# JingruiYu/FishBirdEyeVisualSLAM

Measured on AMD Instinct MI355X. Metric: frames/s (extract+match+pose-opt), 1280x720+512x512 pair, higher is better.
Workload: dtype u8 (extract, Hamming) + f64 (pose optimisation); 1 GPU; configs[2]: 1280x720 front + 512x512 bird pair, HIP ORB extract + M3/M9 Hamming match + PoseOptimizationWithBird (~2k front + ~1k bird edges); nfeatures=2000, parallelism=replicas x1

## Files before the change

### fishbirdeyevisualslam_amd/csrc/orb.hip

```cpp
#include <climits>

#include "fb_common.h"
#include "fb_fast_score.h"
#include "fb_primitives.h"

#include "orb_plan.h"

namespace {

constexpr int PATTERN_XY[1024] = {
#include "orb_pattern.inc"
};
constexpr int pattern_extreme(bool wantMax) {
  int m = PATTERN_XY[0];
  for (int i = 1; i < 1024; i++) m = wantMax ? (PATTERN_XY[i] > m ? PATTERN_XY[i] : m) : (PATTERN_XY[i] < m ? PATTERN_XY[i] : m);
  return m;
}
constexpr int PAT_BIAS = -pattern_extreme(false);
static_assert(PAT_BIAS >= 0 && pattern_extreme(true) + PAT_BIAS <= 255, "a pattern coordinate does not fit a biased byte");
struct PackedPattern { uint32_t test[256]; };
constexpr PackedPattern pack_pattern() {
  PackedPattern p{};
  for (int t = 0; t < 256; t++)
    for (int k = 0; k < 4; k++) p.test[t] |= (uint32_t)(PATTERN_XY[t * 4 + k] + PAT_BIAS) << (8 * k);
  return p;
}
__constant__ PackedPattern c_pattern = pack_pattern();

}

#include "orb_pyramid.inc"
#include "orb_fast.inc"
#include "orb_octree.inc"
#include "orb_describe.inc"

namespace {

struct Workspace {
  int w = 0, h = 0, batchCap = 0;
  OrbK K = {};
  int maxNodes = 0;
  size_t octreeLds = 0;
  bool rowsOK[FB_MAX_LEVELS] = {}, mergeOK[FB_MAX_LEVELS] = {};
  ResizeTabs rt[FB_MAX_LEVELS] = {};
  fb::DevBuf pyr, blur, cand, cellCand, cellCount, nodeOf, counts, lvlOut, tabs, angTab, timers;
};

}

struct fb_orb {
  fb_orb_params p;
  fb_orb_tables t;
  hipStream_t sideStream = nullptr;
  hipEvent_t evFork = nullptr, evJoin = nullptr;
  hipEvent_t evLevel[FB_MAX_LEVELS] = {};
  ~fb_orb() {
    if (evFork) (void)hipEventDestroy(evFork);
    if (evJoin) (void)hipEventDestroy(evJoin);
    for (hipEvent_t e : evLevel)
      if (e) (void)hipEventDestroy(e);
    if (sideStream) (void)hipStreamDestroy(sideStream);
  }
  int kpStride = 0;
  Workspace ws;
  const uint8_t *lastImg = nullptr;
  long long lastImgStride = 0;
  int lastPitch0 = 0;
  fb::DevBuf ownedImg;
};

namespace {

struct OrbCall {
  const uint8_t *img;
  long long imgStride;
  int pitch0, batch;
  hipStream_t s;
};

void launch_resize(fb_orb *o, int l, const OrbCall &c) {
  const Workspace &ws = o->ws;
  const OrbK &K = ws.K;
  const LevelInfo &D = K.L[l], &S = K.L[l - 1];
  const uint8_t *src = (l == 1) ? c.img : ws.pyr.as<uint8_t>() + S.off;
  const long long sstr = (l == 1) ? c.imgStride : K.pyrStride;
  const int spitch = (l == 1) ? c.pitch0 : S.pitch;
  uint8_t *dst = ws.pyr.as<uint8_t>() + D.off;
  const dim3 blk(64, 4);
  auto grid = [&](int rowsPerThread) { return dim3((D.pitch / 4 + 63) / 64, (D.h + 4 * rowsPerThread - 1) / (4 * rowsPerThread), c.batch); };
  fb::ProfScope prof_(fb::P_RESIZE, c.s);
  const bool rows = ws.rowsOK[l] && spitch >= 12 && ((reinterpret_cast<uintptr_t>(src) | (uintptr_t)spitch | (uintptr_t)sstr) & 3) == 0;
  if (rows && ws.mergeOK[l])
    k_resize_merge<<<grid(RM_ROWS), blk, 0, c.s>>>(src, sstr, S.w, S.h, spitch, dst, K.pyrStride, D.w, D.h, D.pitch, ws.rt[l]);
  else if (rows)
    k_resize_rows<<<grid(RESIZE_ROWS), blk, 0, c.s>>>(src, sstr, S.w, S.h, spitch, dst, K.pyrStride, D.w, D.h, D.pitch, ws.rt[l]);
// ... 40 lines not shown
      if (!o->evJoin) FB_HIP(hipEventCreateWithFlags(&o->evJoin, hipEventDisableTiming));
      for (int l = 1; l < FB_MAX_LEVELS; l++)
        if (!o->evLevel[l]) FB_HIP(hipEventCreateWithFlags(&o->evLevel[l], hipEventDisableTiming));
      FB_HIP(hipStreamCreateWithFlags(&o->sideStream, hipStreamNonBlocking));
    }
    sBlur = o->sideStream;
    FB_HIP(hipEventRecord(o->evFork, s));
    FB_HIP(hipStreamWaitEvent(sBlur, o->evFork, 0));
    return FB_OK;
  }

  int behind_level(int l) {
    const int nl = o->ws.K.nlevels;
    if (l + 1 < nl && !((cuts >> (l + 1)) & 1u)) return FB_OK;
    if (fork && l > 0) {
      FB_HIP(hipEventRecord(o->evLevel[l], c.s));
      FB_HIP(hipStreamWaitEvent(sBlur, o->evLevel[l], 0));
    }
    launch_blur(o, c, blurFrom, l + 1, sBlur);
    blurFrom = l + 1;
    if (fork && l + 1 == nl) FB_HIP(hipEventRecord(o->evJoin, sBlur));
    return FB_OK;
  }

  int join_before_describe(hipStream_t s) {
    if (fork) FB_HIP(hipStreamWaitEvent(s, o->evJoin, 0));
    return FB_OK;
  }
};

template <int TP>
void launch_fast(fb_orb *o, const OrbCall &c) {
  const Workspace &ws = o->ws;
  const OrbK &K = ws.K;
  fb::ProfScope prof_(TP == 44 ? fb::P_FAST : TP == 56 ? fb::P_FAST56 : fb::P_FAST72, c.s);
  const dim3 grd((K.totalGroups + 7) / 8 * 8, c.batch);
  const size_t lds = (size_t)2 * K.fastTileBytes + 2 * K.fastMaxPix;
  const auto kern = K.dbg == 20 ? k_fast<TP, true> : k_fast<TP, false>;
  kern<<<grd, 64, lds, c.s>>>(K, c.img, c.imgStride, c.pitch0, ws.pyr.as<uint8_t>(), ws.cellCand.as<uint32_t>(), ws.cellCount.as<int>());
}
void launch_fast(fb_orb *o, const OrbCall &c) {
  const OrbK &K = o->ws.K;
  if (K.totalCells == 0) return;
  if (K.fastTP == 44) launch_fast<44>(o, c);
  else if (K.fastTP == 56) launch_fast<56>(o, c);
  else launch_fast<FAST_MAX_TILE>(o, c);
}

template <int NT>
void launch_octree(fb_orb *o, const OrbCall &c) {
  const Workspace &ws = o->ws;
  int *candCount = ws.counts.as<int>(), *lvlCount = candCount + (size_t)ws.batchCap * ws.K.nlevels;
  fb::ProfScope prof_(fb::P_OCTREE, c.s);
  k_octree<NT><<<dim3(c.batch, ws.K.nlevels), NT, ws.octreeLds, c.s>>>(ws.K, ws.cellCand.as<uint32_t>(), ws.cellCount.as<int>(), ws.cand.as<uint32_t>(), candCount,
                                                                       ws.nodeOf.as<uint16_t>(), ws.lvlOut.as<uint32_t>(), lvlCount, ws.maxNodes);
}
void launch_octree(fb_orb *o, const OrbCall &c) {
  static const int octWideMax = getenv("FB_OCT_WIDE_MAX") ? atoi(getenv("FB_OCT_WIDE_MAX")) : 512;
  if (o->ws.K.nlevels * c.batch <= octWideMax) launch_octree<1024>(o, c);
  else launch_octree<256>(o, c);
}
template <int NT>
int allow_octree_lds() {
  FB_HIP(hipFuncSetAttribute(reinterpret_cast<const void *>(k_octree<NT>), hipFuncAttributeMaxDynamicSharedMemorySize, (int)OCTREE_LDS_MAX));
  return FB_OK;
}

void launch_describe(fb_orb *o, const OrbCall &c, fb_keypoint *d_keypoints, uint8_t *d_descriptors, int32_t *d_n) {
  const Workspace &ws = o->ws;
  const OrbK &K = ws.K;
  const int *lvlCount = ws.counts.as<int>() + (size_t)ws.batchCap * K.nlevels;
  fb::ProfScope prof_(fb::P_DESCRIBE, c.s);
  k_describe<<<dim3((K.descBase[K.nlevels] + 7) / 8 * 8, c.batch), 64 * DESC_WPB, 0, c.s>>>(K, c.img, c.imgStride, c.pitch0, ws.pyr.as<uint8_t>(), ws.blur.as<uint8_t>(),
                                                                                          ws.angTab.as<uint4>(), ws.lvlOut.as<uint32_t>(), lvlCount, d_keypoints,
                                                                                          d_descriptors, d_n);
}

int build_workspace(const OrbPlan &P, int batch, Workspace &ws) {
  ws.K = P.K;
  ws.K.dbg = getenv("FB_FAST_DBG") ? atoi(getenv("FB_FAST_DBG")) : 0;
  ws.maxNodes = P.maxNodes;
  ws.octreeLds = P.octreeLds;
  memcpy(ws.rowsOK, P.rowsOK, sizeof(ws.rowsOK));
  memcpy(ws.mergeOK, P.mergeOK, sizeof(ws.mergeOK));
  FB_TRY(ws.tabs.upload(P.tabBytes.data(), P.tabBytes.size()));
  for (int l = 1; l < P.K.nlevels; l++) {
    const uint8_t *base = ws.tabs.as<uint8_t>();
    ws.rt[l].xofs = reinterpret_cast<const int *>(base + P.tabOff[l][0]);
    ws.rt[l].ialpha = reinterpret_cast<const short *>(base + P.tabOff[l][1]);
    ws.rt[l].yofs = reinterpret_cast<const int *>(base + P.tabOff[l][2]);
    ws.rt[l].ibeta = reinterpret_cast<const short *>(base + P.tabOff[l][3]);
  }
  FB_TRY(ws.angTab.upload(P.angTab, sizeof(P.angTab)));
  const OrbSizes z = P.sizes(batch);
  FB_TRY(ws.pyr.alloc(z.pyr));
  FB_TRY(ws.blur.alloc(z.blur));
  FB_TRY(ws.cand.alloc(z.cand));
  FB_TRY(ws.cellCand.alloc(z.cellCand));
  FB_TRY(ws.cellCount.alloc(z.cellCount));
  FB_TRY(ws.nodeOf.alloc(z.nodeOf));
  FB_TRY(ws.counts.alloc(z.counts));
  FB_TRY(ws.timers.alloc(z.timers));
  FB_HIP(hipMemset(ws.timers.p, 0, z.timers));
  ws.K.timers = ws.timers.as<unsigned long long>();
  FB_TRY(ws.lvlOut.alloc(z.lvlOut));
  return FB_OK;
}

int prepare(fb_orb *o, int w, int h, int batch) {
  if (o->ws.w == w && o->ws.h == h && batch <= o->ws.batchCap) return FB_OK;
  OrbPlan P;
  FB_TRY(plan_orb(o->p, o->t, w, h, o->kpStride, P));
  Workspace ws;
  FB_TRY(build_workspace(P, batch, ws));
  FB_TRY(allow_octree_lds<1024>());
  FB_TRY(allow_octree_lds<256>());
  ws.w = w; ws.h = h; ws.batchCap = batch;
  o->ws = std::move(ws);
  return FB_OK;
}

}

extern "C" {

int fb_orb_capacity(const fb_orb_params *params) {
  if (!params) return FB_ERR_ARG;
  return capacity_of(*params);
}

int fb_orb_set_output_stride(fb_orb *h, int kp_stride) {
  FB_ARG(h && (kp_stride == 0 || kp_stride >= capacity_of(h->p)));
  h->kpStride = kp_stride;
  h->ws.K.kpStride = kp_stride > 0 ? kp_stride : capacity_of(h->p);
  return FB_OK;
// ... 158 lines not shown
```

### fishbirdeyevisualslam_amd/csrc/orb_octree.inc

```

namespace {

__device__ __forceinline__ int quadrant(const ONode &n, int rx, int ry) {
  const int halfX = (int)ceilf((float)(n.x1 - n.x0) / 2), halfY = (int)ceilf((float)(n.y1 - n.y0) / 2);
  const int mx = n.x0 + halfX, my = n.y0 + halfY;
  return (rx < mx ? 0 : 1) + (ry < my ? 0 : 2);
}

__device__ __forceinline__ ONode child_of(const ONode &n, int q, int cnt) {
  const int halfX = (int)ceilf((float)(n.x1 - n.x0) / 2), halfY = (int)ceilf((float)(n.y1 - n.y0) / 2);
  const int mx = n.x0 + halfX, my = n.y0 + halfY;
  ONode c;
  c.x0 = (q & 1) ? mx : n.x0;
  c.x1 = (q & 1) ? n.x1 : mx;
  c.y0 = (q & 2) ? my : n.y0;
  c.y1 = (q & 2) ? n.y1 : my;
  c.cnt = cnt;
  return c;
}

template <int NT>
__global__ __launch_bounds__(NT) void k_octree(OrbK K, const uint32_t *__restrict__ cellCand, const int *__restrict__ cellCount,
                                                uint32_t *__restrict__ cand, int *__restrict__ candCount, uint16_t *__restrict__ nodeOf,
                                                uint32_t *__restrict__ lvlOut, int *__restrict__ lvlCount, int maxNodes) {
  extern __shared__ __attribute__((aligned(16))) uint8_t smem[];
  const int l = blockIdx.y, b = blockIdx.x, tid = threadIdx.x;
  const LevelInfo &Lv = K.L[l];
  const int M = maxNodes;
  ONode *listA = reinterpret_cast<ONode *>(smem);
  ONode *listB = listA + M;
  int *ccnt = reinterpret_cast<int *>(listB + M);
  unsigned short *cpos = reinterpret_cast<unsigned short *>(ccnt + 4 * M);
  unsigned short *npos = cpos + 4 * M;
  unsigned short *order = npos + M;
  unsigned char *split = reinterpret_cast<unsigned char *>(order + M);
  unsigned long long *best = reinterpret_cast<unsigned long long *>(smem + (((size_t)(split + M - smem)) + 7 & ~(size_t)7));
  __shared__ int s_w[NT / 64], s_S, s_nexp, s_jstar;
  uint32_t *cdw = cand + (long long)b * K.candStride + Lv.candBase;
  int n;
  {
    int *offs = reinterpret_cast<int *>(smem);
    const int ncell = Lv.nCols * Lv.nRows;
    const int *cc = cellCount + (long long)b * K.totalCells + Lv.cellBase;
    const uint32_t *sp = cellCand + (long long)b * K.candStride + Lv.candBase;
    int run = 0;
    for (int c0 = 0; c0 < ncell; c0 += NT) {
      const int c = c0 + tid;
      const int v = c < ncell ? cc[c] : 0;
      int tot;
      const int ex = fb::block_excl_scan<NT>(v, s_w, &tot);
      if (c < ncell) offs[c] = run + ex;
      run += tot;
      __syncthreads();
    }
    n = run;
    if (tid == 0) { offs[ncell] = n; candCount[b * K.nlevels + l] = n; }
    __syncthreads();
    for (int k0 = tid; k0 < n; k0 += NT * 4) {
      uint32_t val[4];
#pragma unroll
      for (int u = 0; u < 4; u++) {
        const int k = min(k0 + u * NT, n - 1);
        int lo = 0, hi = ncell;
        while (hi - lo > 1) {
          const int mid = (lo + hi) >> 1;
          if (offs[mid] <= k) lo = mid; else hi = mid;
        }
        val[u] = sp[(long long)lo * Lv.slotCap + (k - offs[lo])];
      }
#pragma unroll
      for (int u = 0; u < 4; u++)
        if (k0 + u * NT < n) cdw[k0 + u * NT] = val[u];
    }
    __threadfence_block();
    __syncthreads();
  }
  const uint32_t *cd = cdw;
  uint16_t *nof = nodeOf + (long long)b * K.candStride + Lv.candBase;
  int *outCount = lvlCount + b * K.nlevels + l;
  uint32_t *out = lvlOut + (long long)b * K.outStride + Lv.outBase;
  if (n == 0 || Lv.nIni < 1) { if (tid == 0) *outCount = 0; return; }
  const int N = Lv.N;
  const int Hh = Lv.h - 2 * BORDER;
  for (int i = tid; i < Lv.nIni; i += NT) {
    ONode nd;
    nd.x0 = (short)(int)(Lv.hX * (float)i);
    nd.x1 = (short)(int)(Lv.hX * (float)(i + 1));
    nd.y0 = 0; nd.y1 = (short)Hh; nd.cnt = 0;
    listB[i] = nd;
  }
  __syncthreads();
  for (int k = tid; k < n; k += NT) {
    const int rx = (int)(cd[k] & 0xFFF) - BORDER;
    int idx = (int)((float)rx / Lv.hX);
    idx = min(idx, Lv.nIni - 1);
    nof[k] = (uint16_t)idx;
    atomicAdd(&listB[idx].cnt, 1);
  }
  __syncthreads();
  if (tid == 0) {
    int S = 0;
    for (int i = 0; i < Lv.nIni; i++) {
      npos[i] = (unsigned short)S;
      if (listB[i].cnt > 0) listA[S++] = listB[i];
    }
    s_S = S;
  }
  __syncthreads();
  for (int k = tid; k < n; k += NT) nof[k] = npos[nof[k]];
  __syncthreads();
  ONode *cur = listA, *nxt = listB;
  int S = s_S;
  bool finalPhase = false;
  for (int guard = 0; guard < 64; guard++) {
    const int prevSize = S;
    for (int i = tid; i < 4 * S; i += NT) ccnt[i] = 0;
    __syncthreads();
    for (int k0 = tid; k0 < n; k0 += NT * 4) {
      int pk[4];
      uint32_t ck[4];
#pragma unroll
      for (int u = 0; u < 4; u++) { const int kk = min(k0 + u * NT, n - 1); pk[u] = nof[kk]; ck[u] = cd[kk]; }
#pragma unroll
      for (int u = 0; u < 4; u++) {
        if (k0 + u * NT >= n) break;
        const int p = pk[u];
        const ONode nd = cur[p];
        if (nd.cnt > 1) {
          const uint32_t c = ck[u];
          atomicAdd(&ccnt[4 * p + quadrant(nd, (int)(c & 0xFFF) - BORDER, (int)((c >> 12) & 0xFFF) - BORDER)], 1);
        }
      }
    }
    __syncthreads();
    if (!finalPhase) {
      for (int p = tid; p < S; p += NT) split[p] = cur[p].cnt > 1;
    } else {
      for (int p = tid; p < S; p += NT) {
        split[p] = 0;
        const int c = cur[p].cnt;
        if (c > 1) {
          int rank = 0;
          for (int j = 0; j < S; j++) {
            const int cj = cur[j].cnt;
            if (cj > 1 && (cj > c || (cj == c && j < p))) rank++;
          }
          order[rank] = (unsigned short)p;
        }
      }
      __syncthreads();
      if (tid == 0) {
        int sz = S, j = 0;
        const int C = s_nexp;
        for (; j < C; j++) {
          const int p = order[j];
          const int kk = (ccnt[4 * p] > 0) + (ccnt[4 * p + 1] > 0) + (ccnt[4 * p + 2] > 0) + (ccnt[4 * p + 3] > 0);
          sz += kk - 1;
          split[p] = 1;
          if (sz >= N) { j++; break; }
        }
        s_jstar = j;
      }
    }
    __syncthreads();
    const int per = (S + NT - 1) / NT;
    const int a0 = min(tid * per, S), a1 = min(a0 + per, S);
    int myKids = 0, myKeep = 0;
    if (!finalPhase) {
      for (int p = a0; p < a1; p++) {
        if (split[p]) myKids += (ccnt[4 * p] > 0) + (ccnt[4 * p + 1] > 0) + (ccnt[4 * p + 2] > 0) + (ccnt[4 * p + 3] > 0);
        else myKeep++;
      }
    } else {
      const int J = s_jstar;
      const int perj = (J + NT - 1) / NT;
      const int r0 = min(tid * perj, J), r1 = min(r0 + perj, J);
      for (int r = r0; r < r1; r++) {
        const int p = order[r];
        myKids += (ccnt[4 * p] > 0) + (ccnt[4 * p + 1] > 0) + (ccnt[4 * p + 2] > 0) + (ccnt[4 * p + 3] > 0);
      }
      for (int p = a0; p < a1; p++) if (!split[p]) myKeep++;
    }
    int totalKids, totalKeep;
    const int kidsBefore = fb::block_excl_scan<NT>(myKids, s_w, &totalKids);
    const int keepBefore = fb::block_excl_scan<NT>(myKeep, s_w, &totalKeep);
    {
      int ci = kidsBefore, kp = totalKids + keepBefore;
      if (!finalPhase) {
        for (int p = a0; p < a1; p++) {
          if (split[p]) {
            for (int q = 0; q < 4; q++)
              if (ccnt[4 * p + q] > 0) {
                const int pos = totalKids - 1 - ci++;
                cpos[4 * p + q] = (unsigned short)pos;
                nxt[pos] = child_of(cur[p], q, ccnt[4 * p + q]);
              }
          } else {
            npos[p] = (unsigned short)kp;
            nxt[kp++] = cur[p];
          }
        }
      } else {
        const int J = s_jstar;
        const int perj = (J + NT - 1) / NT;
        const int r0 = min(tid * perj, J), r1 = min(r0 + perj, J);
        for (int r = r0; r < r1; r++) {
          const int p = order[r];
          for (int q = 0; q < 4; q++)
            if (ccnt[4 * p + q] > 0) {
              const int pos = totalKids - 1 - ci++;
              cpos[4 * p + q] = (unsigned short)pos;
              nxt[pos] = child_of(cur[p], q, ccnt[4 * p + q]);
            }
        }
        for (int p = a0; p < a1; p++)
          if (!split[p]) { npos[p] = (unsigned short)kp; nxt[kp++] = cur[p]; }
      }
    }
    const int Snew = totalKids + totalKeep;
    __syncthreads();
    for (int k0 = tid; k0 < n; k0 += NT * 4) {
      int pk[4];
      uint32_t ck[4];
#pragma unroll
      for (int u = 0; u < 4; u++) { const int kk = min(k0 + u * NT, n - 1); pk[u] = nof[kk]; ck[u] = cd[kk]; }
#pragma unroll
      for (int u = 0; u < 4; u++) {
        const int k = k0 + u * NT;
        if (k >= n) break;
        const int p = pk[u];
        if (split[p]) {
          const uint32_t c = ck[u];
          nof[k] = cpos[4 * p + quadrant(cur[p], (int)(c & 0xFFF) - BORDER, (int)((c >> 12) & 0xFFF) - BORDER)];
        } else nof[k] = npos[p];
      }
    }
    int myExp = 0;
    {
      const int pern = (Snew + NT - 1) / NT;
      const int n0 = min(tid * pern, Snew), n1 = min(n0 + pern, Snew);
      for (int p = n0; p < n1; p++) myExp += (p < totalKids && nxt[p].cnt > 1);
    }
    int nToExpand;
    fb::block_excl_scan<NT>(myExp, s_w, &nToExpand);
    if (tid == 0) s_nexp = nToExpand;
    __syncthreads();
    ONode *t = cur; cur = nxt; nxt = t;
    S = Snew;
    if (S >= N || S == prevSize) break;
    if (!finalPhase) {
      if (S + nToExpand * 3 > N) finalPhase = true;
    }
  }
  for (int p = tid; p < S; p += NT) best[p] = 0ull;
  __syncthreads();
  for (int k0 = tid; k0 < n; k0 += NT * 4) {
    int pk[4];
    uint32_t ck[4];
#pragma unroll
    for (int u = 0; u < 4; u++) { const int kk = min(k0 + u * NT, n - 1); pk[u] = nof[kk]; ck[u] = cd[kk]; }
#pragma unroll
    for (int u = 0; u < 4; u++) {
    const int k = k0 + u * NT;
    if (k >= n) break;
    const uint32_t c = ck[u];
    const int x = c & 0xFFF, y = (c >> 12) & 0xFFF, r = c >> 24;
    const int cellI = (y - EDGE_THRESHOLD) / Lv.hCell, cellJ = (x - EDGE_THRESHOLD) / Lv.wCell;
    const int dwid = min(Lv.wCell, Lv.w - 2 * EDGE_THRESHOLD - cellJ * Lv.wCell);
    const int inCell = (y - EDGE_THRESHOLD - cellI * Lv.hCell) * dwid + (x - EDGE_THRESHOLD - cellJ * Lv.wCell);
    const unsigned orderKey = (unsigned)(cellI * Lv.nCols + cellJ) * 4096u + (unsigned)inCell;
    const unsigned long long key = ((unsigned long long)r << 56) | ((unsigned long long)(0xFFFFFFFFu - orderKey) << 24) | (unsigned)k;
    atomicMax(&best[pk[u]], key);
    }
  }
  __syncthreads();
  for (int p = tid; p < S; p += NT) out[p] = cd[(unsigned)(best[p] & 0xFFFFFFull)];
  if (tid == 0) *outCount = S;
}

}
```

### fishbirdeyevisualslam_amd/csrc/orb_plan.h

```cpp
#ifndef FB_ORB_PLAN_H_
#define FB_ORB_PLAN_H_

#include <algorithm>
#include <cstdint>
#include <cstring>
#include <vector>

#include "../../include/fishbird.h"

#ifndef FB_HD
#define FB_HD
#endif
#include "fb_detmath.h"

namespace fb {
void set_error(const char *fmt, ...);
}

namespace {

constexpr int EDGE_THRESHOLD = 19;
constexpr int HALF_PATCH = 15;
constexpr int PATCH_SIZE = 31;
constexpr int BORDER = EDGE_THRESHOLD - 3;

constexpr int FAST_MAX_TILE = 72;
constexpr int FAST_CPW = 4;
constexpr int DESC_WPB = 4;
constexpr int DESC_KPW = 2;
constexpr int BLUR_ROWS = 32;
constexpr size_t OCTREE_LDS_MAX = 160 * 1024 - 512;
#ifdef FB_FAST_LISTHIST
#define FB_ORB_TIMER_WORDS (16 + 128)
#else
#define FB_ORB_TIMER_WORDS 16
#endif

struct LevelInfo {
  int w, h, pitch;
  long long off;
  int nCols, nRows, wCell, hCell, cellBase;
  int N;
  long long candBase;
  int candCap;
  int slotCap;
  int outBase, outCap;
  int nIni;
  float hX;
  float scale;
  int patchSize;
  long long boff;
};

struct OrbK {
  int nlevels, iniTh, minTh, totalCells, outStride, capOut;
  int kpStride;
  int fastTileBytes, fastMaxOut, fastMaxPix;
  int fastTP;
  int dbg;
  unsigned long long *timers;
  int cellBase[FB_MAX_LEVELS + 1];
  int grpBase[FB_MAX_LEVELS + 1];
  int totalGroups;
  int descBase[FB_MAX_LEVELS + 1];
  int runBase[FB_MAX_LEVELS];
  int runCap[FB_MAX_LEVELS];
  long long pyrStride;
  long long blurStride;
  int blurStrips[FB_MAX_LEVELS + 1];
  long long candStride;
  int umax[16];
  LevelInfo L[FB_MAX_LEVELS];
};

struct ResizeTabs {
  const int *xofs;
  const short *ialpha;
  const int *yofs;
  const short *ibeta;
};

struct ONode {
  short x0, y0, x1, y1;
  int cnt;
};

inline void make_tables(const fb_orb_params &p, fb_orb_tables &t) {
  memset(&t, 0, sizeof(t));
  const int nl = p.nlevels;
  t.scale_factor[0] = 1.0f;
  t.level_sigma2[0] = 1.0f;
  for (int i = 1; i < nl; i++) {
    t.scale_factor[i] = t.scale_factor[i - 1] * p.scale_factor;
    t.level_sigma2[i] = t.scale_factor[i] * t.scale_factor[i];
  }
  for (int i = 0; i < nl; i++) {
    t.inv_scale_factor[i] = 1.0f / t.scale_factor[i];
    t.inv_level_sigma2[i] = 1.0f / t.level_sigma2[i];
  }
  float factor = 1.0f / p.scale_factor;
  float nDesired = p.nfeatures * (1 - factor) / (1 - (float)pow((double)factor, (double)nl));
  int sum = 0;
  for (int l = 0; l < nl - 1; l++) {
    t.features_per_level[l] = fb_cvround(nDesired);
    sum += t.features_per_level[l];
    nDesired *= factor;
  }
  t.features_per_level[nl - 1] = std::max(p.nfeatures - sum, 0);
  int umax[HALF_PATCH + 2] = {0};
  int v, v0;
  const int vmax = fb_cvfloor(HALF_PATCH * sqrtf(2.f) / 2 + 1);
  const int vmin = fb_cvceil(HALF_PATCH * sqrtf(2.f) / 2);
  const double hp2 = HALF_PATCH * HALF_PATCH;
  for (v = 0; v <= vmax; ++v) umax[v] = fb_cvround_d(sqrt(hp2 - v * v));
  for (v = HALF_PATCH, v0 = 0; v >= vmin; --v) {
    while (umax[v0] == umax[v0 + 1]) ++v0;
    umax[v] = v0;
    ++v0;
  }
  for (int i = 0; i <= HALF_PATCH; i++) t.umax[i] = umax[i];
}

inline int capacity_of(const fb_orb_params &p) { return p.nfeatures + 8 * p.nlevels; }

struct OrbSizes {
  size_t pyr, blur, cand, cellCand, cellCount, nodeOf, counts, lvlOut, timers;
};

struct OrbPlan {
  OrbK K;
  bool rowsOK[FB_MAX_LEVELS];
  bool mergeOK[FB_MAX_LEVELS];
  std::vector<uint8_t> tabBytes;
  size_t tabOff[FB_MAX_LEVELS][4];
  uint32_t angTab[64 * 4];
  int maxNodes;
  size_t octreeLds;
  OrbSizes sizes(size_t B) const {
    OrbSizes z;
    z.pyr = B * K.pyrStride + 256;
    z.blur = B * K.blurStride + 256;
    z.cand = z.cellCand = B * K.candStride * 4 + 16;
    z.cellCount = B * (size_t)K.totalCells * 4 + 16;
    z.nodeOf = B * K.candStride * 2 + 16;
    z.counts = B * K.nlevels * 4 * 2 + FB_MAX_LEVELS * 4;
    z.lvlOut = B * K.outStride * 4 + 16;
    z.timers = FB_ORB_TIMER_WORDS * 8;
    return z;
  }
};

inline int plan_level(const fb_orb_params &p, const fb_orb_tables &t, int w, int h, int l, LevelInfo &L) {
  const float scale = t.inv_scale_factor[l];
  L.w = fb_cvround((float)w * scale);
  L.h = fb_cvround((float)h * scale);
  if (l == 0) { L.w = w; L.h = h; }
  if (L.w < 1 || L.h < 1) {
    fb::set_error("pyramid level %d of a %dx%d image is empty (scale factor %.3f, %d levels)", l, w, h, (double)p.scale_factor, p.nlevels);
    return FB_ERR_ARG;
  }
  if (L.w >= 4096 || L.h >= 4096) { fb::set_error("image too large (level %d is %dx%d, limit 4095)", l, L.w, L.h); return FB_ERR_ARG; }
  L.pitch = (L.w + 63) & ~63;
  const int maxBX = L.w - BORDER, maxBY = L.h - BORDER;
  const float width = (float)(maxBX - BORDER), height = (float)(maxBY - BORDER);
  L.nCols = (int)(width / 30.f);
  L.nRows = (int)(height / 30.f);
  if (L.nCols <= 0 || L.nRows <= 0) { L.nCols = L.nRows = 0; L.wCell = L.hCell = 1; }
  else { L.wCell = (int)ceilf(width / L.nCols); L.hCell = (int)ceilf(height / L.nRows); }
  if (L.wCell + 6 > FAST_MAX_TILE - 3 || L.hCell + 6 > FAST_MAX_TILE) { fb::set_error("FAST cell %dx%d exceeds the LDS tile", L.wCell, L.hCell); return FB_ERR_CAPACITY; }
  if (L.nCols * L.nRows >= (1 << 20)) { fb::set_error("level %d has more than 2^20 FAST cells", l); return FB_ERR_CAPACITY; }
  L.N = t.features_per_level[l];
  L.slotCap = ((L.wCell + 1) / 2) * ((L.hCell + 1) / 2);
  L.candCap = L.nCols * L.nRows * L.slotCap + 16;
  if (L.candCap >= (1 << 24)) { fb::set_error("level %d: more than 2^24 FAST candidates possible", l); return FB_ERR_CAPACITY; }
  const int Wr = maxBX - BORDER, Hr = maxBY - BORDER;
  L.nIni = (Hr > 0) ? (int)roundf((float)Wr / Hr) : 0;
  L.hX = L.nIni > 0 ? (float)Wr / L.nIni : 1.f;
  L.outCap = std::max(L.N + 3, 4 * L.nIni) + 4;
  L.scale = t.scale_factor[l];
  L.patchSize = (int)(PATCH_SIZE * t.scale_factor[l]);
  return FB_OK;
}

inline void plan_offsets(OrbPlan &P) {
  OrbK &K = P.K;
  long long pyrOff = 0, candOff = 0, blurOff = 0;
  int cells = 0, outOff = 0, strips = 0;
  P.maxNodes = 0;
  for (int l = 0; l < K.nlevels; l++) {
    LevelInfo &L = K.L[l];
// ... 62 lines not shown
    int sy = fb_cvfloor(fy);
    fy -= sy;
    yofs[dy] = sy;
    ibeta[dy * 2] = (short)fb_cvround((1.f - fy) * 2048.f);
    ibeta[dy * 2 + 1] = (short)fb_cvround(fy * 2048.f);
  }
  P.rowsOK[l] = resize_rows_ok(xofs);
  P.mergeOK[l] = P.rowsOK[l] && resize_merge_ok(yofs);
  auto append = [&](const void *src, size_t n) {
    const size_t off = (P.tabBytes.size() + 15) & ~(size_t)15;
    P.tabBytes.resize(off + n);
    memcpy(P.tabBytes.data() + off, src, n);
    return off;
  };
  P.tabOff[l][0] = append(xofs.data(), xofs.size() * 4);
  P.tabOff[l][1] = append(ialpha.data(), ialpha.size() * 2);
  P.tabOff[l][2] = append(yofs.data(), yofs.size() * 4);
  P.tabOff[l][3] = append(ibeta.data(), ibeta.size() * 2);
}

inline void plan_fast_tile(OrbK &K) {
  int tileB = 0, maxOut = 0, maxPix = 0, tpNeed = 0;
  for (int l = 0; l < K.nlevels; l++) {
    const LevelInfo &L = K.L[l];
    if (L.nCols * L.nRows == 0) continue;
    const int tpMax = (L.wCell + 6 + 3 + 3) & ~3, chMax = L.hCell + 6;
    tpNeed = std::max(tpNeed, tpMax);
    tileB = std::max(tileB, chMax);
    maxOut = std::max(maxOut, L.slotCap);
    maxPix = std::max(maxPix, L.wCell * L.hCell);
  }
  K.fastTP = tpNeed <= 44 ? 44 : tpNeed <= 56 ? 56 : FAST_MAX_TILE;
  K.fastTileBytes = (std::max(K.fastTP * tileB, 4 * ((maxOut + 3) & ~3)) + 15) & ~15;
  K.fastTileBytes = std::max(K.fastTileBytes, (21 * K.fastTP + 15) & ~15);
  K.fastMaxOut = (maxOut + 3) & ~3;
  K.fastMaxPix = (maxPix + 7) & ~7;
}

inline void plan_grids(OrbK &K) {
  int gsum = 0, wsum = 0;
  for (int l = 0; l <= FB_MAX_LEVELS; l++) {
    K.cellBase[l] = l < K.nlevels ? K.L[l].cellBase : K.totalCells;
    K.grpBase[l] = gsum;
    K.descBase[l] = wsum;
    if (l >= K.nlevels) continue;
    gsum += (K.L[l].nCols * K.L[l].nRows + FAST_CPW - 1) / FAST_CPW;
    K.runBase[l] = K.L[l].outBase;
    K.runCap[l] = K.L[l].outCap;
    wsum += (K.L[l].outCap + DESC_WPB * DESC_KPW - 1) / (DESC_WPB * DESC_KPW);
  }
  K.totalGroups = gsum;
}

inline int plan_octree_lds(OrbPlan &P) {
  const size_t M = P.maxNodes;
  size_t lds = 2 * M * sizeof(ONode) + 4 * M * 4 + 4 * M * 2 + M * 2 + M * 2 + M;
  lds = ((lds + 7) & ~(size_t)7) + M * 8 + 16;
  size_t maxCells = 0;
  for (int l = 0; l < P.K.nlevels; l++) maxCells = std::max(maxCells, (size_t)P.K.L[l].nCols * P.K.L[l].nRows);
  lds = std::max(lds, (maxCells + 1) * 4 + 16);
  if (lds > OCTREE_LDS_MAX) { fb::set_error("nfeatures too large for the LDS quadtree (%zu B)", lds); return FB_ERR_CAPACITY; }
  P.octreeLds = lds;
  return FB_OK;
}

inline void plan_angle_table(OrbPlan &P) {
  for (int lane = 0; lane < 62; lane++) {
    const int v = (lane >> 1) - 15, half = lane & 1, dmax = P.K.umax[v < 0 ? -v : v];
    for (int j = 0; j < 16; j++) {
      const int au = half ? j : 15 - j;
      const bool inc = au <= dmax && (half || au != 0);
      if (!inc) continue;
      P.angTab[lane * 4 + (j >> 2)] |= ((uint32_t)au | 0x10u) << (8 * (j & 3));
    }
  }
}

inline int plan_orb(const fb_orb_params &p, const fb_orb_tables &t, int w, int h, int kpStride, OrbPlan &out) {
  OrbPlan P;
  memset(&P.K, 0, sizeof(P.K));
  memset(P.rowsOK, 0, sizeof(P.rowsOK));
  memset(P.mergeOK, 0, sizeof(P.mergeOK));
  memset(P.tabOff, 0, sizeof(P.tabOff));
  memset(P.angTab, 0, sizeof(P.angTab));
  OrbK &K = P.K;
  K.nlevels = p.nlevels;
  K.iniTh = p.ini_th_fast;
  K.minTh = p.min_th_fast;
  K.capOut = capacity_of(p);
  K.kpStride = kpStride > 0 ? kpStride : K.capOut;
  for (int i = 0; i < 16; i++) K.umax[i] = t.umax[i];
  for (int l = 0; l < p.nlevels; l++) {
    const int rc = plan_level(p, t, w, h, l, K.L[l]);
    if (rc != FB_OK) return rc;
  }
  plan_offsets(P);
  for (int l = 1; l < p.nlevels; l++) plan_resize_tables(P, l);
  plan_fast_tile(K);
  plan_grids(K);
  const int rc = plan_octree_lds(P);
  if (rc != FB_OK) return rc;
  plan_angle_table(P);
  out = std::move(P);
  return FB_OK;
}

}

#endif
```

Before: 81590 frames/s.

## Keep octree candidates and node ids in LDS, fuse quadrant counting into remap

The quadtree distribution kernel now copies each level's candidates and node indices into LDS when they fit (up to 8192 candidates by default), so the per-round passes no longer read and write global memory. Quadrant counting for the next round is folded into the remap pass, removing one pass over the candidates per round. The serial choose loop run by thread 0 in the final phase is replaced by a block-wide scan with an atomicMin cutoff. Per-phase timers sit behind a template flag, and probe scripts are added. The cost is much more LDS per workgroup, which can lower occupancy, plus two code paths to maintain.

```diff
diff --git a/fishbirdeyevisualslam_amd/csrc/orb.hip b/fishbirdeyevisualslam_amd/csrc/orb.hip
--- a/fishbirdeyevisualslam_amd/csrc/orb.hip
+++ b/fishbirdeyevisualslam_amd/csrc/orb.hip
@@ -41,6 +41,7 @@
   OrbK K = {};
   int maxNodes = 0;
   size_t octreeLds = 0;
+  int octreeCand = 0, octreeCandNarrow = 0, octreeCandOff = 0;
   bool rowsOK[FB_MAX_LEVELS] = {}, mergeOK[FB_MAX_LEVELS] = {};
   ResizeTabs rt[FB_MAX_LEVELS] = {};
   fb::DevBuf pyr, blur, cand, cellCand, cellCount, nodeOf, counts, lvlOut, tabs, angTab, timers;
@@ -187,8 +188,11 @@
   const Workspace &ws = o->ws;
   int *candCount = ws.counts.as<int>(), *lvlCount = candCount + (size_t)ws.batchCap * ws.K.nlevels;
   fb::ProfScope prof_(fb::P_OCTREE, c.s);
-  k_octree<NT><<<dim3(c.batch, ws.K.nlevels), NT, ws.octreeLds, c.s>>>(ws.K, ws.cellCand.as<uint32_t>(), ws.cellCount.as<int>(), ws.cand.as<uint32_t>(), candCount,
-                                                                       ws.nodeOf.as<uint16_t>(), ws.lvlOut.as<uint32_t>(), lvlCount, ws.maxNodes);
+  const auto kern = ws.K.dbg >= 21 && ws.K.dbg < 21 + FB_MAX_LEVELS ? k_octree<NT, true> : k_octree<NT, false>;
+  const int cand = NT == 1024 ? ws.octreeCand : ws.octreeCandNarrow;
+  const size_t lds = (size_t)ws.octreeCandOff + (size_t)cand * 6;
+  kern<<<dim3(c.batch, ws.K.nlevels), NT, lds, c.s>>>(ws.K, ws.cellCand.as<uint32_t>(), ws.cellCount.as<int>(), ws.cand.as<uint32_t>(), candCount,
+                                                                       ws.nodeOf.as<uint16_t>(), ws.lvlOut.as<uint32_t>(), lvlCount, ws.maxNodes, cand, ws.octreeCandOff);
 }
 void launch_octree(fb_orb *o, const OrbCall &c) {
   static const int octWideMax = getenv("FB_OCT_WIDE_MAX") ? atoi(getenv("FB_OCT_WIDE_MAX")) : 512;
@@ -197,7 +201,8 @@
 }
 template <int NT>
 int allow_octree_lds() {
-  FB_HIP(hipFuncSetAttribute(reinterpret_cast<const void *>(k_octree<NT>), hipFuncAttributeMaxDynamicSharedMemorySize, (int)OCTREE_LDS_MAX));
+  FB_HIP(hipFuncSetAttribute(reinterpret_cast<const void *>(k_octree<NT, false>), hipFuncAttributeMaxDynamicSharedMemorySize, (int)OCTREE_LDS_MAX));
+  FB_HIP(hipFuncSetAttribute(reinterpret_cast<const void *>(k_octree<NT, true>), hipFuncAttributeMaxDynamicSharedMemorySize, (int)OCTREE_LDS_MAX));
   return FB_OK;
 }
 
@@ -215,7 +220,11 @@
   ws.K = P.K;
   ws.K.dbg = getenv("FB_FAST_DBG") ? atoi(getenv("FB_FAST_DBG")) : 0;
   ws.maxNodes = P.maxNodes;
-  ws.octreeLds = P.octreeLds;
+  const char *oc = getenv("FB_OCT_LDS_CAND");
+  ws.octreeCand = oc ? std::max(0, std::min(atoi(oc), P.octreeCandMax)) : P.octreeCand;
+  ws.octreeCandNarrow = oc ? ws.octreeCand : 0;
+  ws.octreeCandOff = (int)P.octreeNodeLds;
+  ws.octreeLds = octree_lds_bytes(P, ws.octreeCand);
   memcpy(ws.rowsOK, P.rowsOK, sizeof(ws.rowsOK));
   memcpy(ws.mergeOK, P.mergeOK, sizeof(ws.mergeOK));
   FB_TRY(ws.tabs.upload(P.tabBytes.data(), P.tabBytes.size()));
diff --git a/fishbirdeyevisualslam_amd/csrc/orb_octree.inc b/fishbirdeyevisualslam_amd/csrc/orb_octree.inc
--- a/fishbirdeyevisualslam_amd/csrc/orb_octree.inc
+++ b/fishbirdeyevisualslam_amd/csrc/orb_octree.inc
@@ -19,67 +19,34 @@
   return c;
 }
 
-template <int NT>
-__global__ __launch_bounds__(NT) void k_octree(OrbK K, const uint32_t *__restrict__ cellCand, const int *__restrict__ cellCount,
-                                                uint32_t *__restrict__ cand, int *__restrict__ candCount, uint16_t *__restrict__ nodeOf,
-                                                uint32_t *__restrict__ lvlOut, int *__restrict__ lvlCount, int maxNodes) {
-  extern __shared__ __attribute__((aligned(16))) uint8_t smem[];
-  const int l = blockIdx.y, b = blockIdx.x, tid = threadIdx.x;
-  const LevelInfo &Lv = K.L[l];
-  const int M = maxNodes;
-  ONode *listA = reinterpret_cast<ONode *>(smem);
-  ONode *listB = listA + M;
-  int *ccnt = reinterpret_cast<int *>(listB + M);
-  unsigned short *cpos = reinterpret_cast<unsigned short *>(ccnt + 4 * M);
-  unsigned short *npos = cpos + 4 * M;
-  unsigned short *order = npos + M;
-  unsigned char *split = reinterpret_cast<unsigned char *>(order + M);
-  unsigned long long *best = reinterpret_cast<unsigned long long *>(smem + (((size_t)(split + M - smem)) + 7 & ~(size_t)7));
-  __shared__ int s_w[NT / 64], s_S, s_nexp, s_jstar;
-  uint32_t *cdw = cand + (long long)b * K.candStride + Lv.candBase;
-  int n;
-  {
-    int *offs = reinterpret_cast<int *>(smem);
-    const int ncell = Lv.nCols * Lv.nRows;
-    const int *cc = cellCount + (long long)b * K.totalCells + Lv.cellBase;
-    const uint32_t *sp = cellCand + (long long)b * K.candStride + Lv.candBase;
-    int run = 0;
-    for (int c0 = 0; c0 < ncell; c0 += NT) {
-      const int c = c0 + tid;
-      const int v = c < ncell ? cc[c] : 0;
-      int tot;
-      const int ex = fb::block_excl_scan<NT>(v, s_w, &tot);
-      if (c < ncell) offs[c] = run + ex;
-      run += tot;
-      __syncthreads();
-    }
-    n = run;
-    if (tid == 0) { offs[ncell] = n; candCount[b * K.nlevels + l] = n; }
-    __syncthreads();
-    for (int k0 = tid; k0 < n; k0 += NT * 4) {
-      uint32_t val[4];
-#pragma unroll
-      for (int u = 0; u < 4; u++) {
-        const int k = min(k0 + u * NT, n - 1);
-        int lo = 0, hi = ncell;
-        while (hi - lo > 1) {
-          const int mid = (lo + hi) >> 1;
-          if (offs[mid] <= k) lo = mid; else hi = mid;
-        }
-        val[u] = sp[(long long)lo * Lv.slotCap + (k - offs[lo])];
-      }
-#pragma unroll
-      for (int u = 0; u < 4; u++)
-        if (k0 + u * NT < n) cdw[k0 + u * NT] = val[u];
-    }
-    __threadfence_block();
-    __syncthreads();
-  }
-  const uint32_t *cd = cdw;
-  uint16_t *nof = nodeOf + (long long)b * K.candStride + Lv.candBase;
-  int *outCount = lvlCount + b * K.nlevels + l;
-  uint32_t *out = lvlOut + (long long)b * K.outStride + Lv.outBase;
-  if (n == 0 || Lv.nIni < 1) { if (tid == 0) *outCount = 0; return; }
+struct OctLds {
+  ONode *listA, *listB;
+  int *ccnt;
+  unsigned short *cpos;
+  unsigned short *npos;
+  unsigned short *order;
+  unsigned char *split;
+  unsigned long long *best;
+};
+
+template <bool TIMED>
+struct OctTimer {
+  uint32_t mark = 0, start = 0, acc[7] = {0, 0, 0, 0, 0, 0, 0};
+  int rounds = 0;
+};
+template <>
+struct OctTimer<false> {};
+
+template <int NT, bool TIMED, bool RES, typename CandPtr, typename NodePtr>
+__device__ __forceinline__ int octree_rounds(const LevelInfo &Lv, const OctLds D, CandPtr cd, NodePtr nof, int n, uint32_t *__restrict__ out, int *s_w, int *s_S,
+                                             int *s_nexp, int *s_jstar, bool timed, OctTimer<TIMED> &T) {
+#define OCT_TICK(slot_) if constexpr (TIMED) if (timed) { __builtin_amdgcn_sched_barrier(0); const uint32_t t_ = (uint32_t)__builtin_amdgcn_s_memtime(); __builtin_amdgcn_sched_barrier(0); T.acc[slot_] += t_ - T.mark; T.mark = t_; }
+  const int tid = threadIdx.x;
+  ONode *listA = D.listA, *listB = D.listB;
+  int *ccnt = D.ccnt;
+  unsigned short *cpos = D.cpos, *npos = D.npos, *order = D.order;
+  unsigned char *split = D.split;
+  unsigned long long *best = D.best;
   const int N = Lv.N;
   const int Hh = Lv.h - 2 * BORDER;
   for (int i = tid; i < Lv.nIni; i += NT) {
@@ -104,35 +71,53 @@
       npos[i] = (unsigned short)S;
       if (listB[i].cnt > 0) listA[S++] = listB[i];
     }
-    s_S = S;
-  }
-  __syncthreads();
-  for (int k = tid; k < n; k += NT) nof[k] = npos[nof[k]];
-  __syncthreads();
+    *s_S = S;
+  }
+  __syncthreads();
+  if constexpr (RES) {
+    for (int i = tid; i < 4 * *s_S; i += NT) ccnt[i] = 0;
+    __syncthreads();
+    for (int k = tid; k < n; k += NT) {
+      const int p = npos[nof[k]];
+      nof[k] = (uint16_t)p;
+      const ONode nd = listA[p];
+      if (nd.cnt > 1) {
+        const uint32_t c = cd[k];
+        atomicAdd(&ccnt[4 * p + quadrant(nd, (int)(c & 0xFFF) - BORDER, (int)((c >> 12) & 0xFFF) - BORDER)], 1);
+      }
+    }
+  } else {
+    for (int k = tid; k < n; k += NT) nof[k] = npos[nof[k]];
+  }
+  __syncthreads();
+  OCT_TICK(1)
   ONode *cur = listA, *nxt = listB;
-  int S = s_S;
+  int S = *s_S;
   bool finalPhase = false;
   for (int guard = 0; guard < 64; guard++) {
     const int prevSize = S;
-    for (int i = tid; i < 4 * S; i += NT) ccnt[i] = 0;
-    __syncthreads();
-    for (int k0 = tid; k0 < n; k0 += NT * 4) {
-      int pk[4];
-      uint32_t ck[4];
-#pragma unroll
-      for (int u = 0; u < 4; u++) { const int kk = min(k0 + u * NT, n - 1); pk[u] = nof[kk]; ck[u] = cd[kk]; }
-#pragma unroll
-      for (int u = 0; u < 4; u++) {
-        if (k0 + u * NT >= n) break;
-        const int p = pk[u];
-        const ONode nd = cur[p];
-        if (nd.cnt > 1) {
-          const uint32_t c = ck[u];
-          atomicAdd(&ccnt[4 * p + quadrant(nd, (int)(c & 0xFFF) - BORDER, (int)((c >> 12) & 0xFFF) - BORDER)], 1);
-        }
-      }
-    }
-    __syncthreads();
+    if constexpr (!RES) {
+      for (int i = tid; i < 4 * S; i += NT) ccnt[i] = 0;
+      __syncthreads();
+      for (int k0 = tid; k0 < n; k0 += NT * 4) {
+        int pk[4];
+        uint32_t ck[4];
+#pragma unroll
+        for (int u = 0; u < 4; u++) { const int kk = min(k0 + u * NT, n - 1); pk[u] = nof[kk]; ck[u] = cd[kk]; }
+#pragma unroll
+        for (int u = 0; u < 4; u++) {
+          if (k0 + u * NT >= n) break;
+          const int p = pk[u];
+          const ONode nd = cur[p];
+          if (nd.cnt > 1) {
+            const uint32_t c = ck[u];
+            atomicAdd(&ccnt[4 * p + quadrant(nd, (int)(c & 0xFFF) - BORDER, (int)((c >> 12) & 0xFFF) - BORDER)], 1);
+          }
+        }
+      }
+      __syncthreads();
+    }
+    OCT_TICK(2)
     if (!finalPhase) {
       for (int p = tid; p < S; p += NT) split[p] = cur[p].cnt > 1;
     } else {
@@ -149,9 +134,29 @@
         }
       }
       __syncthreads();
-      if (tid == 0) {
+      if constexpr (RES) {
+        const int C = *s_nexp;
+        const int perc = (C + NT - 1) / NT;
+        const int r0 = min(tid * perc, C), r1 = min(r0 + perc, C);
+        int mine = 0;
+        for (int r = r0; r < r1; r++) {
+          const int p = order[r];
+          mine += (ccnt[4 * p] > 0) + (ccnt[4 * p + 1] > 0) + (ccnt[4 * p + 2] > 0) + (ccnt[4 * p + 3] > 0) - 1;
+        }
+        if (tid == 0) *s_jstar = C;
+        int tot;
+        int sz = S + fb::block_excl_scan<NT>(mine, s_w, &tot);
+        if (sz < N)
+          for (int r = r0; r < r1; r++) {
+            const int p = order[r];
+            sz += (ccnt[4 * p] > 0) + (ccnt[4 * p + 1] > 0) + (ccnt[4 * p + 2] > 0) + (ccnt[4 * p + 3] > 0) - 1;
+            if (sz >= N) { atomicMin(s_jstar, r + 1); break; }
+          }
+        __syncthreads();
+        for (int r = tid; r < *s_jstar; r += NT) split[order[r]] = 1;
+      } else if (tid == 0) {
         int sz = S, j = 0;
-        const int C = s_nexp;
+        const int C = *s_nexp;
         for (; j < C; j++) {
           const int p = order[j];
           const int kk = (ccnt[4 * p] > 0) + (ccnt[4 * p + 1] > 0) + (ccnt[4 * p + 2] > 0) + (ccnt[4 * p + 3] > 0);
@@ -159,10 +164,11 @@
           split[p] = 1;
           if (sz >= N) { j++; break; }
         }
-        s_jstar = j;
-      }
-    }
-    __syncthreads();
+        *s_jstar = j;
+      }
+    }
+    __syncthreads();
+    OCT_TICK(3)
     const int per = (S + NT - 1) / NT;
     const int a0 = min(tid * per, S), a1 = min(a0 + per, S);
     int myKids = 0, myKeep = 0;
@@ -172,7 +178,7 @@
         else myKeep++;
       }
     } else {
-      const int J = s_jstar;
+      const int J = *s_jstar;
       const int perj = (J + NT - 1) / NT;
       const int r0 = min(tid * perj, J), r1 = min(r0 + perj, J);
       for (int r = r0; r < r1; r++) {
@@ -201,7 +207,7 @@
           }
         }
       } else {
-        const int J = s_jstar;
+        const int J = *s_jstar;
         const int perj = (J + NT - 1) / NT;
         const int r0 = min(tid * perj, J), r1 = min(r0 + perj, J);
         for (int r = r0; r < r1; r++) {
@@ -219,22 +225,10 @@
     }
     const int Snew = totalKids + totalKeep;
     __syncthreads();
-    for (int k0 = tid; k0 < n; k0 += NT * 4) {
-      int pk[4];
-      uint32_t ck[4];
-#pragma unroll
-      for (int u = 0; u < 4; u++) { const int kk = min(k0 + u * NT, n - 1); pk[u] = nof[kk]; ck[u] = cd[kk]; }
-#pragma unroll
-      for (int u = 0; u < 4; u++) {
-        const int k = k0 + u * NT;
-        if (k >= n) break;
-        const int p = pk[u];
-        if (split[p]) {
-          const uint32_t c = ck[u];
-          nof[k] = cpos[4 * p + quadrant(cur[p], (int)(c & 0xFFF) - BORDER, (int)((c >> 12) & 0xFFF) - BORDER)];
-        } else nof[k] = npos[p];
-      }
-    }
+    OCT_TICK(4)
+    const bool countNext = RES && !(Snew >= N || Snew == prevSize);
+    if (countNext)
+      for (int i = tid; i < 4 * Snew; i += NT) ccnt[i] = 0;
     int myExp = 0;
     {
       const int pern = (Snew + NT - 1) / NT;
@@ -242,9 +236,34 @@
       for (int p = n0; p < n1; p++) myExp += (p < totalKids && nxt[p].cnt > 1);
     }
     int nToExpand;
-    fb::block_excl_scan<NT>(myExp, s_w, &nToExpand);
-    if (tid == 0) s_nexp = nToExpand;
-    __syncthreads();
+    if constexpr (RES) fb::block_excl_scan<NT>(myExp, s_w, &nToExpand);
+    for (int k0 = tid; k0 < n; k0 += NT * 4) {
+      int pk[4];
+      uint32_t ck[4];
+#pragma unroll
+      for (int u = 0; u < 4; u++) { const int kk = min(k0 + u * NT, n - 1); pk[u] = nof[kk]; ck[u] = cd[kk]; }
+#pragma unroll
+      for (int u = 0; u < 4; u++) {
+        const int k = k0 + u * NT;
+        if (k >= n) break;
+        const int p = pk[u];
+        const uint32_t c = ck[u];
+        const int rx = (int)(c & 0xFFF) - BORDER, ry = (int)((c >> 12) & 0xFFF) - BORDER;
+        int np;
+        if (split[p]) np = cpos[4 * p + quadrant(cur[p], rx, ry)];
+        else np = npos[p];
+        nof[k] = (uint16_t)np;
+        if (countNext) {
+          const ONode nd = nxt[np];
+          if (nd.cnt > 1) atomicAdd(&ccnt[4 * np + quadrant(nd, rx, ry)], 1);
+        }
+      }
+    }
+    if constexpr (!RES) fb::block_excl_scan<NT>(myExp, s_w, &nToExpand);
+    if (tid == 0) *s_nexp = nToExpand;
+    __syncthreads();
+    OCT_TICK(5)
+    if constexpr (TIMED) T.rounds++;
     ONode *t = cur; cur = nxt; nxt = t;
     S = Snew;
     if (S >= N || S == prevSize) break;
@@ -275,7 +294,104 @@
   }
   __syncthreads();
   for (int p = tid; p < S; p += NT) out[p] = cd[(unsigned)(best[p] & 0xFFFFFFull)];
+  OCT_TICK(6)
+#undef OCT_TICK
+  return S;
+}
+
+template <int NT, bool TIMED>
+__global__ __launch_bounds__(NT) void k_octree(OrbK K, const uint32_t *__restrict__ cellCand, const int *__restrict__ cellCount,
+                                                uint32_t *__restrict__ cand, int *__restrict__ candCount, uint16_t *__restrict__ nodeOf,
+                                                uint32_t *__restrict__ lvlOut, int *__restrict__ lvlCount, int maxNodes, int ldsCand, int candOff) {
+  extern __shared__ __attribute__((aligned(16))) uint8_t smem[];
+  const int l = blockIdx.y, b = blockIdx.x, tid = threadIdx.x;
+  const LevelInfo &Lv = K.L[l];
+  const int M = maxNodes;
+  OctLds D;
+  D.listA = reinterpret_cast<ONode *>(smem);
+  D.listB = D.listA + M;
+  D.ccnt = reinterpret_cast<int *>(D.listB + M);
+  D.cpos = reinterpret_cast<unsigned short *>(D.ccnt + 4 * M);
+  D.npos = D.cpos + 4 * M;
+  D.order = D.npos + M;
+  D.split = reinterpret_cast<unsigned char *>(D.order + M);
+  D.best = reinterpret_cast<unsigned long long *>(smem + (((size_t)(D.split + M - smem)) + 7 & ~(size_t)7));
+  uint32_t *lcand = reinterpret_cast<uint32_t *>(smem + candOff);
+  uint16_t *lnode = reinterpret_cast<uint16_t *>(lcand + ldsCand);
+  __shared__ int s_w[NT / 64], s_S, s_nexp, s_jstar;
+  const bool timed = TIMED && tid == 0 && l == K.dbg - 21;
+  OctTimer<TIMED> T;
+  if constexpr (TIMED) {
+    if (timed) { __builtin_amdgcn_sched_barrier(0); T.mark = (uint32_t)__builtin_amdgcn_s_memtime(); __builtin_amdgcn_sched_barrier(0); }
+    T.start = T.mark;
+  }
+  uint32_t *cdw = cand + (long long)b * K.candStride + Lv.candBase;
+  int n;
+  bool res;
+  {
+    int *offs = reinterpret_cast<int *>(smem);
+    const int ncell = Lv.nCols * Lv.nRows;
+    const int *cc = cellCount + (long long)b * K.totalCells + Lv.cellBase;
+    const uint32_t *sp = cellCand + (long long)b * K.candStride + Lv.candBase;
+    int run = 0;
+    for (int c0 = 0; c0 < ncell; c0 += NT) {
+      const int c = c0 + tid;
+      const int v = c < ncell ? cc[c] : 0;
+      int tot;
+      const int ex = fb::block_excl_scan<NT>(v, s_w, &tot);
+      if (c < ncell) offs[c] = run + ex;
+      run += tot;
+      __syncthreads();
+    }
+    n = run;
+    res = n <= ldsCand;
+    if (tid == 0) { offs[ncell] = n; candCount[b * K.nlevels + l] = n; }
+    __syncthreads();
+    for (int k0 = tid; k0 < n; k0 += NT * 4) {
+      uint32_t val[4];
+#pragma unroll
+      for (int u = 0; u < 4; u++) {
+        const int k = min(k0 + u * NT, n - 1);
+        int lo = 0, hi = ncell;
+        while (hi - lo > 1) {
+          const int mid = (lo + hi) >> 1;
+          if (offs[mid] <= k) lo = mid; else hi = mid;
+        }
+        val[u] = sp[(long long)lo * Lv.slotCap + (k - offs[lo])];
+      }
+#pragma unroll
+      for (int u = 0; u < 4; u++)
+        if (k0 + u * NT < n) {
+          cdw[k0 + u * NT] = val[u];
+          if (res) lcand[k0 + u * NT] = val[u];
+        }
+    }
+    __threadfence_block();
+    __syncthreads();
+  }
+  if constexpr (TIMED)
+    if (timed) { __builtin_amdgcn_sched_barrier(0); const uint32_t t_ = (uint32_t)__builtin_amdgcn_s_memtime(); __builtin_amdgcn_sched_barrier(0); T.acc[0] += t_ - T.mark; T.mark = t_; }
+  int *outCount = lvlCount + b * K.nlevels + l;
+  uint32_t *out = lvlOut + (long long)b * K.outStride + Lv.outBase;
+  if (n == 0 || Lv.nIni < 1) { if (tid == 0) *outCount = 0; return; }
+  int S;
+  if (res) {
+    S = octree_rounds<NT, TIMED, true>(Lv, D, (const uint32_t *)lcand, lnode, n, out, s_w, &s_S, &s_nexp, &s_jstar, timed, T);
+  } else {
+    const uint32_t *cd = cdw;
+    uint16_t *nof = nodeOf + (long long)b * K.candStride + Lv.candBase;
+    S = octree_rounds<NT, TIMED, false>(Lv, D, cd, nof, n, out, s_w, &s_S, &s_nexp, &s_jstar, timed, T);
+  }
   if (tid == 0) *outCount = S;
-}
-
-}
+  if constexpr (TIMED) if (timed) {
+#pragma unroll
+    for (int i = 0; i < 7; i++) atomicAdd(&K.timers[i], (unsigned long long)T.acc[i]);
+    atomicAdd(&K.timers[7], (unsigned long long)(T.mark - T.start));
+    atomicAdd(&K.timers[8], 1ull);
+    atomicAdd(&K.timers[9], (unsigned long long)T.rounds);
+    atomicAdd(&K.timers[10], (unsigned long long)n);
+    atomicAdd(&K.timers[11], res ? 1ull : 0ull);
+  }
+}
+
+}
diff --git a/fishbirdeyevisualslam_amd/csrc/orb_plan.h b/fishbirdeyevisualslam_amd/csrc/orb_plan.h
--- a/fishbirdeyevisualslam_amd/csrc/orb_plan.h
+++ b/fishbirdeyevisualslam_amd/csrc/orb_plan.h
@@ -30,6 +30,7 @@
 constexpr int DESC_KPW = 2;
 constexpr int BLUR_ROWS = 32;
 constexpr size_t OCTREE_LDS_MAX = 160 * 1024 - 512;
+constexpr int OCTREE_LDS_CAND = 8192;
 #ifdef FB_FAST_LISTHIST
 #define FB_ORB_TIMER_WORDS (16 + 128)
 #else
@@ -136,6 +137,9 @@
   uint32_t angTab[64 * 4];
   int maxNodes;
   size_t octreeLds;
+  size_t octreeNodeLds;
+  int octreeCand;
+  int octreeCandMax;
   OrbSizes sizes(size_t B) const {
     OrbSizes z;
     z.pyr = B * K.pyrStride + 256;
@@ -304,6 +308,7 @@
   K.totalGroups = gsum;
 }
 
+inline size_t octree_lds_bytes(const OrbPlan &P, int cand) { return P.octreeNodeLds + (size_t)cand * 6; }
 inline int plan_octree_lds(OrbPlan &P) {
   const size_t M = P.maxNodes;
   size_t lds = 2 * M * sizeof(ONode) + 4 * M * 4 + 4 * M * 2 + M * 2 + M * 2 + M;
@@ -312,7 +317,13 @@
   for (int l = 0; l < P.K.nlevels; l++) maxCells = std::max(maxCells, (size_t)P.K.L[l].nCols * P.K.L[l].nRows);
   lds = std::max(lds, (maxCells + 1) * 4 + 16);
   if (lds > OCTREE_LDS_MAX) { fb::set_error("nfeatures too large for the LDS quadtree (%zu B)", lds); return FB_ERR_CAPACITY; }
-  P.octreeLds = lds;
+  int maxCand = 0;
+  for (int l = 0; l < P.K.nlevels; l++) maxCand = std::max(maxCand, P.K.L[l].candCap);
+  const size_t nodeLds = std::min((lds + 15) & ~(size_t)15, OCTREE_LDS_MAX);
+  P.octreeNodeLds = nodeLds;
+  P.octreeCandMax = (int)std::min<size_t>((OCTREE_LDS_MAX - nodeLds) / 6, (size_t)std::min(maxCand, 65532)) & ~3;
+  P.octreeCand = std::min(OCTREE_LDS_CAND, P.octreeCandMax);
+  P.octreeLds = octree_lds_bytes(P, P.octreeCand);
   return FB_OK;
 }
 
diff --git a/profiles/probes/kernel_stats_table.py b/profiles/probes/kernel_stats_table.py
--- /dev/null
+++ b/profiles/probes/kernel_stats_table.py
@@ -0,0 +1,9 @@
+import csv
+import re
+import sys
+
+for r in csv.DictReader(open(sys.argv[1])):
+    name = r["Name"].replace("(anonymous namespace)::", "").replace("void ", "")
+    m = re.match(r"[A-Za-z_0-9:]+(<[^>(]*>)?", name)
+    print("%-34s calls %4s  avg %9.1f us  min %9.1f  max %9.1f  %5s %%" % (m.group(0)[:34], r["Calls"], float(r["AverageNs"]) / 1e3, float(r["MinNs"]) / 1e3,
+                                                                       float(r["MaxNs"]) / 1e3, r["Percentage"][:5]))
diff --git a/profiles/probes/octree_phase_timers.py b/profiles/probes/octree_phase_timers.py
--- /dev/null
+++ b/profiles/probes/octree_phase_timers.py
@@ -0,0 +1,34 @@
+import sys, os, ctypes as C
+sys.path.insert(0, '.')
+import numpy as np, torch
+import fishbirdeyevisualslam_amd as fb
+from fishbirdeyevisualslam_amd import synth, cabi
+from fishbirdeyevisualslam_amd.pipeline import FramePipeline
+lvl = int(os.environ.get("FB_FAST_DBG", "0")) - 21
+assert 0 <= lvl < 8
+B = int(sys.argv[1]) if len(sys.argv) > 1 else 256
+R = min(B, 16)
+f = np.stack([synth.synth_image(1000 + i, 1280, 720) for i in range(R)] * (B // R))
+b = np.stack([synth.synth_image(1500 + i, 512, 512) for i in range(R)] * (B // R))
+pipe = FramePipeline(B)
+pipe.set_images(f, b)
+L = fb.lib()
+s = C.c_void_p(torch.cuda.current_stream().cuda_stream)
+for _ in range(3): pipe.extract(s)
+torch.cuda.synchronize()
+names = ["pack", "initial nodes", "count", "choose", "rebuild", "remap", "best per node"]
+print("B = %d, level %d" % (B, lvl))
+for which, orb in (("front", pipe.orb_f), ("bird", pipe.orb_b)):
+    t = (C.c_uint64 * 16)()
+    fb.check(L.fb_orb_debug_timers(orb, t), "timers")
+    pipe.extract(s); torch.cuda.synchronize()
+    fb.check(L.fb_orb_debug_timers(orb, t), "timers")
+    n = max(t[8], 1)
+    print("%s: %d workgroups timed, %.0f ticks each, %.1f rounds, %.0f candidates" % (which, t[8], t[7] / n, t[9] / n, t[10] / n))
+    for i in range(7):
+        print("   %-16s %8.0f ticks  %5.1f %%" % (names[i], t[i] / n, 100.0 * t[i] / max(t[7], 1)))
+L.fb_prof_reset(); L.fb_prof_enable(1)
+for _ in range(5): pipe.extract(s)
+torch.cuda.synchronize()
+ents = (cabi.ProfEntry * 32)(); n = L.fb_prof_report(ents, 32)
+print("kernel ms per extract of front + bird (timed instantiation):", {ents[i].name.decode(): round(ents[i].total_ms / 5, 3) for i in range(n) if "oct" in ents[i].name.decode()})
```

Result: no change. 81450 frames/s (-0.2%).
